# Ogeon/pyrite

Measured on AMD Instinct MI355X. Metric: Msamples/sec, higher is better.
Workload: dtype f32; 1 GPU; C3: c3_mesh_in_box, 1920x1080, 1024 spp; bounces=8, light_samples=4, spectrum_samples=10, spectrum_bins=64, tile_size=32, triangles=819212, spheres=0, parallelism=one launch on one GPU, film_weight_check=ok

## Files before the change

### pyrite_amd/build.py

```python
import os
import subprocess
import sys

CSRC = os.path.join(os.path.dirname(os.path.abspath(__file__)), "csrc")
OUT = os.path.join(CSRC, "libpyrite_gpu.so")
KERNELS = os.path.join(CSRC, "kernels")
KERNEL_UNITS = ["main.hip", "interp.hip", "product.hip", "wide.hip", "film.hip", "features.hip", "features_wide.hip", "tone.hip", "denoise.hip", "build.hip", "refit.hip"]
PROFILE_UNIT = "profile.hip"
PLAIN_UNITS = ["film.hip", "features.hip", "features_wide.hip", "tone.hip", "denoise.hip", "build.hip", "refit.hip"]
SOURCES = ["api.cpp", "multi.cpp", "bvh.cpp", "bvh_device.cpp", "program_regs.cpp"]
HEADERS = ["kernels.hip", "bvh.h", "bvh_level.h", "bvh_device.h", "device_scene.h", "api_internal.h", "exact_math.h", "program_regs.h", os.path.join("..", "..", "include", "pyrite_gpu.h")]
HIPCC = os.environ.get("HIPCC", "/opt/rocm/bin/hipcc")
FLAGS = [
    "-O3", "-std=c++17", "--offload-arch=gfx950", "-fPIC", "-shared",
    "-munsafe-fp-atomics",
    "-fno-fast-math",
    "-ffp-contract=off",
    "-Wall", "-Wno-unused-function",
    "-mllvm", "-disable-vector-combine",
    "-fno-slp-vectorize",
]


def stale():
    if not os.path.exists(OUT):
        return True
    t = os.path.getmtime(OUT)
    files = [os.path.join(CSRC, f) for f in SOURCES + HEADERS] + [os.path.join(KERNELS, f) for f in os.listdir(KERNELS)]
    return os.path.getmtime(os.path.abspath(__file__)) > t or any(os.path.getmtime(f) > t for f in files)


IMAGES_OUT = os.path.join(CSRC, "libpyrite_images.so")


def build_images(force=False, verbose=False):
    src = os.path.join(CSRC, "jpeg.c")
    if not force and os.path.exists(IMAGES_OUT) and os.path.getmtime(IMAGES_OUT) >= os.path.getmtime(src):
        return IMAGES_OUT
    cmd = [os.environ.get("CC", "gcc"), "-O2", "-fPIC", "-shared", "-Wall", "-o", IMAGES_OUT, src, "-lm"]
    if verbose:
        print(" ".join(cmd))
    subprocess.check_call(cmd, cwd=CSRC)
    return IMAGES_OUT

# ... 83 lines not shown
```

### pyrite_amd/csrc/device_scene.h

```cpp
#pragma once
#include <cstddef>
#include <cstdint>

#include "../../include/pyrite_gpu.h"

namespace pyr {

struct DevPrim {
    float a[4], b[4], c[4];
};

struct DevPrimPair {
    float q[5][4];
};

struct DevTriShade {
    float n1[4], n2[4], n3[4];
};

struct DevTriTex {
    float uv12[4], uv3[4], f1[4], f2[4], f3[4];
};

struct DevTexture {
// ... 88 lines not shown
constexpr uint32_t tape_rows_needed(uint32_t n_spectral, bool rgb) {
    return (rgb ? tape_rgb_row(n_spectral) + 3u : (n_spectral == 0u ? 0u : tape_row(n_spectral - 1u) + 1u)) > kTapeValueRows
               ? (rgb ? tape_rgb_row(n_spectral) + 3u : tape_row(n_spectral - 1u) + 1u)
               : kTapeValueRows;
}

constexpr uint32_t kMaxStackDepth = 64;

struct RenderLaunch {
    PyrCamera camera;
    PyrFilmDesc film;
    uint32_t bounces, light_samples, spectrum_samples, tile_size, pixel_samples;
    uint32_t tiles_x, tiles_y;
    uint32_t tile_begin, tile_stride, tile_count;
    uint32_t chunks_per_tile;
    uint32_t chunk_begin, chunk_end;
    uint32_t film_layout;
    uint32_t film_row_begin, film_row_count;
    uint64_t seed;
    float grains_per_wavelength;
    PyrGrain* film_out;
    unsigned long long* counters;
    uint32_t scheduler;
    uint32_t sm_phase_lanes, sm_trav_steps;
    uint32_t sm_expose_lanes;
    uint32_t stack_lds;
    unsigned long long* tape;
    uint32_t tape_lanes, tape_max_ops;
    uint32_t* tape_overflow;
    uint32_t tape_programs_lds;
    uint32_t sample_begin;
    uint32_t* start_queue;
    uint32_t start_queue_stride;
};

#ifndef PYR_SAMPLE_QUEUE
#define PYR_SAMPLE_QUEUE 1
#endif
constexpr uint32_t kStartQueueEntries = 128, kStartQueueFixedWords = 11;
constexpr uint32_t start_queue_words(uint32_t spectrum_samples) { return kStartQueueFixedWords + spectrum_samples; }

constexpr uint32_t kFeedSegments = 8, kFeedCursorStride = 64;
constexpr size_t kFeedBytes = (size_t)kFeedSegments * kFeedCursorStride * sizeof(uint32_t);

struct IntersectLaunch {
    const float* rays;
    PyrHit* hits;
    uint32_t n;
    unsigned long long* counters;
    uint32_t* next;
    uint32_t num_cus;
    uint32_t reserve;
    uint32_t stack_lds;
};

struct DevelopLaunch {
    PyrFilmDesc film;
    const PyrGrain* grains;
    float step_size, xyz_scale;
    uint32_t sample_count;
    const float* filter;
    const float* white_div;
    const float* white_mul;
    const float* xyz_table;
    uint32_t xyz_count;
    float xyz_min, xyz_max;
// ... 90 lines not shown
```

### pyrite_amd/csrc/kernels.hip

```cpp
#ifndef PYRITE_KERNELS_HIP
#define PYRITE_KERNELS_HIP
#include <hip/hip_runtime.h>

#include <algorithm>
#include <cstdint>
#include <cstdlib>
#include <string>
#include <type_traits>

#include "device_scene.h"
#include "exact_math.h"

#ifdef PYR_WIDE_VM
#define PYR_VM_NUMBERS PYR_WIDE_NUMBER_REGISTERS
#define PYR_VM_VECTORS PYR_WIDE_VECTOR_REGISTERS
#define PYR_VM_RGBS PYR_WIDE_RGB_REGISTERS
#else
#define PYR_VM_NUMBERS PYR_MAX_NUMBER_REGISTERS
#define PYR_VM_VECTORS PYR_MAX_VECTOR_REGISTERS
#define PYR_VM_RGBS PYR_MAX_RGB_REGISTERS
#endif
static_assert((PYR_VM_NUMBERS & (PYR_VM_NUMBERS - 1)) == 0 && (PYR_VM_VECTORS & (PYR_VM_VECTORS - 1)) == 0 && (PYR_VM_RGBS & (PYR_VM_RGBS - 1)) == 0,
              "the interpreter masks register indices: its files are powers of two");

namespace pyr {
#ifdef PYR_WIDE_VM
namespace wide {
#endif

#define DEV __device__ __forceinline__
DEV unsigned long long ballot64(bool p) { return __builtin_amdgcn_ballot_w64(p); }

constexpr int BLOCK = 256;
#ifndef PYR_SM_WAVES
#define PYR_SM_WAVES 4
#endif
constexpr float DIST_EPSILON = 0.0001f;
constexpr float PI_F = 3.14159265358979323846f;
#define PYR_INF __builtin_huge_valf()

struct f3 {
    float x, y, z;
};
DEV f3 mk(float x, float y, float z) { return f3{x, y, z}; }
// ... 1196 lines not shown
        spec.wl(hero) = spec.wl(SS - 1);
        if constexpr (COMPANION_STATE)
            for (uint32_t k = 0; k + 1 < SS; ++k) {
                spec.bright(k) = 0.0f;
                spec.refl(k) = 1.0f;
            }
    }
    p.bright = 0.0f;
    p.refl = 1.0f;
    p.use_additional = true;
    p.sample_light = true;
    p.events = 0;
    p.bounce = 0;
}

DEV bool locate_chunk(const RenderLaunch& L, uint32_t chunk, uint32_t lane, uint32_t& tile, uint64_t& iteration, TileArea& area) {
    const uint32_t k = chunk / L.chunks_per_tile, within = chunk - k * L.chunks_per_tile;
    tile = L.tile_begin + k * L.tile_stride;
    const uint32_t ty = tile / L.tiles_x, tx = tile - ty * L.tiles_x;
    const uint32_t sx = tx * L.tile_size, sy = ty * L.tile_size;
    const uint32_t w = min(L.film.width - sx, L.tile_size), h = min(L.film.height - sy, L.tile_size);
    const uint64_t area_px = (uint64_t)w * h, iterations = area_px * L.pixel_samples;
    iteration = (uint64_t)within * 64u + lane;
    if (iteration >= iterations) return false;
    iteration += area_px * L.sample_begin;
    area = to_view_area(sx, sy, w, h, L.film.width, L.film.height);
    return true;
}

struct SyncProf {
    unsigned long long section[8] = {0, 0, 0, 0, 0, 0, 0, 0}, last = 0;
};
#ifdef PYR_PHASE_PROFILE
__device__ unsigned long long g_phase_prof[16];
#define SLAP(sp, i)                                 \
    {                                               \
        const unsigned long long now_ = clock64();  \
        (sp).section[i] += now_ - (sp).last;        \
        (sp).last = now_;                           \
    }
#else
#define SLAP(sp, i)
#endif

constexpr int SYNC_PRIO_T = 3, SYNC_PRIO_N = 2, SYNC_PRIO_S = 1, SYNC_PRIO_E = 0;
#define SYNC_PRIO(x) __builtin_amdgcn_s_setprio(x)
template <bool COUNT>
DEV bool bounce_step(const DevScene& S, const RenderLaunch& L, const SceneView& view, Path& p, Spectral& spec, int* stack, Counters& cnt, SyncProf& sp) {
    const uint32_t n_add = L.spectrum_samples - 1;
    Hit hit;
    if (COUNT) cnt.extension_rays++;
    const f3 ray_o = p.o, ray_d = p.d;
    SYNC_PRIO(SYNC_PRIO_T);
    const bool found = traverse<COUNT, false>(S, view.nodes, view.prims, ray_o, ray_d, 0.0f, hit, stack, cnt);
    SYNC_PRIO(SYNC_PRIO_S);
    SLAP(sp, 1);
    if (!found) {
        uint32_t color = S.sky_program;
        if (p.sample_light) {
            for (uint32_t i = 0; i < S.num_lamps; ++i) {
                const DevLamp& l = S.lamps[i];
                if (l.kind == PYR_LAMP_DIRECTIONAL && dot(ld3(l.v), ray_d) >= l.width) {
                    color = l.color_program;
                    break;
                }
            }
        }
// ... 213 lines not shown
        uint32_t tile;
        uint64_t iteration;
        TileArea area;
        if (!locate_chunk(L, chunk, lane, tile, iteration, area)) continue;
        Path p{};
        start_sample(launch_from_kernarg(L), tile, iteration, area, p, spec);
        if (COUNT) cnt.samples++;
        SLAP(sp, 0);
        while (p.bounce < L.bounces) {
            const bool ended = bounce_step<COUNT>(S, launch_from_kernarg(L), view, p, spec, stack, cnt, sp);
            p.bounce++;
            if (ended) break;
        }
        SLAP(sp, 6);
        SYNC_PRIO(SYNC_PRIO_E);
        finish_path<COUNT>(launch_from_kernarg(L), p, spec, cnt);
        SLAP(sp, 7);
    }
#ifdef PYR_PHASE_PROFILE
    if (lane == 0)
        for (int i = 0; i < 8; ++i) atomicAdd(&g_phase_prof[i], sp.section[i]);
#endif
    flush_counters<COUNT>(cnt, L.counters);
}

#ifdef PYR_PHASE_PROFILE
#define PROF_DECL unsigned long long prof_c[4] = {0, 0, 0, 0}, prof_l[4] = {0, 0, 0, 0}, prof_n[4] = {0, 0, 0, 0}
#define PROF_BEGIN(ph, cond) const unsigned long long prof_t0_##ph = clock64(); prof_l[ph] += __popcll(ballot64(cond)); prof_n[ph]++
#define PROF_END(ph) prof_c[ph] += clock64() - prof_t0_##ph
#define PROF_LANES(ph, cond) prof_l[ph] += __popcll(ballot64(cond)); prof_n[ph]++
#define PROF_NOW() clock64()
#define PROF_EXTRA(idx, cycles) if ((threadIdx.x & 63u) == 0) atomicAdd(&g_phase_prof[idx], (unsigned long long)(cycles))
#define PROF_ADD(acc, v) (acc) += (v)
#define PROF_FLUSH()                                                                                  \
    if ((threadIdx.x & 63u) == 0)                                                                     \
        for (int i = 0; i < 4; ++i) {                                                                 \
            atomicAdd(&g_phase_prof[i], prof_c[i]);                                                   \
            atomicAdd(&g_phase_prof[4 + i], prof_l[i]);                                               \
            atomicAdd(&g_phase_prof[8 + i], prof_n[i]);                                               \
        }
#else
#define PROF_DECL
#define PROF_BEGIN(ph, cond)
#define PROF_END(ph)
#define PROF_LANES(ph, cond)
#define PROF_NOW() 0ull
#define PROF_EXTRA(idx, cycles)
#define PROF_ADD(acc, v)
#define PROF_FLUSH()
#endif

enum Stage : uint32_t { ST_NEW = 0, ST_TRAV = 1, ST_SHADE = 2, ST_NEE = 3, ST_EXPOSE = 4, ST_DONE = 5 };

struct Trav {
    f3 o, d, inv;
    uint32_t nx = 0, ny = 0, nz = 0;
    float limit, closest;
    int node, sp;
    uint32_t shape;
    float u, v;
    bool shadow, blocked;
};

DEV void trav_ray_signs(Trav& t) {
    t.nx = (__float_as_uint(t.d.x) >> 31) * 48u;
    t.ny = (__float_as_uint(t.d.y) >> 31) * 48u;
    t.nz = (__float_as_uint(t.d.z) >> 31) * 48u;
}
DEV float shadow_cutoff(float limit, float margin) { return __builtin_amdgcn_sqrtf(limit * margin + 1.0e-3f); }
DEV void trav_restart(Trav& t, float shadow_margin) {
    if (t.shadow) t.closest = shadow_cutoff(t.limit, shadow_margin);
    t.blocked = false;
    t.node = 0;
    t.sp = 0;
}

template <bool COUNT>
DEV bool trav_begin(const DevScene& S, Trav& t, f3 o, f3 d, bool shadow, float limit, Counters& cnt) {
    t.o = o;
    t.d = d;
    t.shadow = shadow;
// ... 339 lines not shown
    const uint32_t* tape_prepared = nullptr;
    DEV void tape_push(const RenderLaunch& L, uint32_t kind, uint32_t program, float s, bool hero_only = false) {
        if (n_ops < L.tape_max_ops) {
            uint32_t word = (kind << 30) | (hero_only ? TAPE_HERO_ONLY : 0u) | (program & TAPE_PROGRAM_MASK);
            if (tape_prepared != nullptr) {
                uint32_t slot = kTapeOneSlot;
                if (kind != TAPE_SCALE) {
                    const uint32_t* e = tape_prepared + 8 * program;
                    if (e[0] == 0u)
                        s = __uint_as_float(e[1]) * s;
                    else
                        slot = e[7];
                }
                word = (kind == TAPE_ADD ? TAPE_EAGER_ADD : 0u) | (hero_only ? TAPE_HERO_ONLY : 0u) | (slot << TAPE_EAGER_SLOT_SHIFT);
            }
            L.tape[tape_index(n_ops, L.tape_lanes, tape_column)] = (unsigned long long)word | ((unsigned long long)__float_as_uint(s) << 32);
        } else {
            *L.tape_overflow = 1u;
        }
        n_ops++;
    }
    DEV void tape_push_raw(const RenderLaunch& L, uint32_t word, float s) {
        if (n_ops < L.tape_max_ops)
            L.tape[tape_index(n_ops, L.tape_lanes, tape_column)] = (unsigned long long)word | ((unsigned long long)__float_as_uint(s) << 32);
        else
            *L.tape_overflow = 1u;
        n_ops++;
    }
    uint32_t rgb_slot = 0;
    static constexpr bool QUEUE = PYR_SAMPLE_QUEUE != 0 && TAPE && !INTERP;
    uint32_t chunk = 0;
    uint32_t q_state = 0;
#ifdef PYR_PHASE_PROFILE
    unsigned long long prof_start[4] = {0, 0, 0, 0};
#endif
    Path p{};
    Trav t{};
    f3 b_position = mk(0, 0, 0), b_normal = mk(0, 0, 0), b_out = mk(0, 0, 0);
    bool b_flip = false;
    DEV f3 b_nff() const { return b_flip ? -b_normal : b_normal; }
    bool b_has_brdf = false;
    uint32_t nee_lamp = 0, nee_i = 0;
    DEV static float nee_probability(const DevScene& S, const RenderLaunch& L) {
        const float lamp_probability = 1.0f / (float)S.num_lamps;
        return 1.0f / ((float)L.light_samples * 2.0f * PI_F * lamp_probability);
    }
    bool ls_pending = false, ls_physical = false;
    uint32_t ls_material = 0, ls_color = 0;
    f3 ls_normal = mk(0, 0, 0);
    float ls_scale = 0.0f;
    float ls_tx = 0.0f, ls_ty = 0.0f;

    enum : uint32_t { CONTRIB_NONE = 0, CONTRIB_MUL = 1, CONTRIB_ADD = 2 };
    uint32_t c_kind = CONTRIB_NONE, c_color = 0;
    int c_probability = -1;
    float c_cp = 1.0f, c_outer = 1.0f, c_scale = 1.0f;
    bool c_use_outer = false, c_companions = false, c_has_scale = false;
    f3 c_normal = mk(0, 0, 0), c_incident = mk(0, 0, 0);
    float c_tx = 0.0f, c_ty = 0.0f;
    DEV void contribution(uint32_t kind, uint32_t color, int probability, float cp, bool use_outer, float outer, bool companions, f3 normal, f3 incident, float tx,
                          float ty) {
        c_kind = kind, c_color = color, c_probability = probability, c_cp = cp, c_use_outer = use_outer, c_outer = outer, c_companions = companions;
        c_normal = normal, c_incident = incident, c_tx = tx, c_ty = ty;
    }
    DEV void contribution_clear() {
        c_kind = CONTRIB_NONE, c_color = 0u, c_probability = -1;
// ... 460 lines not shown
    for (uint32_t k = 0; k < p.num_instrs; ++k) {
        const PyrInstr& ins = S.instrs[p.first_instr + k];
        float r = 0.0f;
        switch (ins.op) {
        case PYR_OP_NUMBER: r = __uint_as_float(ins.x.bits); break;
        case PYR_OP_SPECTRUM: r = spectrum_get(S, ins.a, value(ins.x)); break;
        case PYR_OP_BLACKBODY: {
            const float wl = value(ins.x), temp = value(ins.y);
            r = blackbody(wl, temp);
            break;
        }
        case PYR_OP_MIX: {
            const float amount = fmaxf(fminf(value(ins.x), 1.0f), 0.0f);
            const float l = num[ins.a & (PYR_MAX_NUMBER_REGISTERS - 1)], rr = num[ins.b & (PYR_MAX_NUMBER_REGISTERS - 1)];
            r = l * (1.0f - amount) + rr * amount;
            break;
        }
        case PYR_OP_BINARY: {
            const float l = num[ins.a & (PYR_MAX_NUMBER_REGISTERS - 1)], rr = num[ins.b & (PYR_MAX_NUMBER_REGISTERS - 1)];
            r = ins.operator_ == PYR_BIN_ADD ? l + rr : (ins.operator_ == PYR_BIN_SUB ? l - rr : (ins.operator_ == PYR_BIN_MUL ? l * rr : l / rr));
            break;
        }
        default: {
            const float v = value(ins.x), mn = value(ins.y), mx = value(ins.z);
            r = fmaxf(fminf(v, mx), mn);
            break;
        }
        }
        num[ins.output & (PYR_MAX_NUMBER_REGISTERS - 1)] = r;
    }
    return num[p.output_reg & (PYR_MAX_NUMBER_REGISTERS - 1)];
}

template <bool COUNT, bool RGB = false, bool TIMES = false>
DEV void replay_tapes(const DevScene& S, const RenderLaunch& L, bool exposing, uint32_t n_ops, uint32_t tape_column, const Path& p, const float* wl_rows,
                      uint32_t wl_column, uint32_t* wave_list, const uint32_t* prepared_lds, float* spectral_values, uint32_t n_spectral, bool eager, Counters& cnt) {
    const uint32_t lane = threadIdx.x & 63u;
    const unsigned long long mask = ballot64(exposing);
    const uint32_t n = (uint32_t)__popcll(mask);
    if (n == 0) return;
    uint32_t max_ops = exposing ? (n_ops < L.tape_max_ops ? n_ops : L.tape_max_ops) : 0u;
    const uint32_t my_ops = max_ops;
    for (int off = 32; off > 0; off >>= 1) max_ops = max(max_ops, (uint32_t)__shfl_xor((int)max_ops, off));
    const bool keeps = exposing && p.use_additional, lost = exposing && !p.use_additional;
    const bool longest = 3u * my_ops > 2u * max_ops, shortest = 3u * my_ops <= max_ops;
    const unsigned long long below = (1ull << lane) - 1ull;
    const unsigned long long k0 = ballot64(keeps && longest), k1 = ballot64(keeps && !longest && !shortest), k2 = ballot64(keeps && shortest);
    const unsigned long long l0 = ballot64(lost && longest), l1 = ballot64(lost && !longest && !shortest), l2 = ballot64(lost && shortest);
    const uint32_t n_full = (uint32_t)__builtin_popcountll(k0 | k1 | k2);
    if (exposing) {
        const unsigned long long mine = keeps ? (longest ? k0 : (shortest ? k2 : k1)) : (longest ? l0 : (shortest ? l2 : l1));
        uint32_t before = keeps ? 0u : n_full;
        before += (uint32_t)__builtin_popcountll(keeps ? ((longest ? 0ull : k0) | (shortest ? k1 : 0ull)) : ((longest ? 0ull : l0) | (shortest ? l1 : 0ull)));
        wave_list[before + (uint32_t)__builtin_popcountll(mine & below)] = lane;
    }
    __builtin_amdgcn_wave_barrier();
    const uint32_t SS = L.spectrum_samples, full_items = n_full * SS, items = full_items + (n - n_full);
    const unsigned long long past_the_end =
        eager ? ((unsigned long long)(kTapeOneSlot << TAPE_EAGER_SLOT_SHIFT) | ((unsigned long long)__float_as_uint(1.0f) << 32)) : 0ull;
#ifndef PYR_REPLAY_ROWS
#define PYR_REPLAY_ROWS 8
#endif
    constexpr uint32_t ROWS = PYR_REPLAY_ROWS;
    for (uint32_t base = 0; base < items; base += 64) {
        const uint32_t i = base + lane;
        const bool active = i < items;
        const bool full = i < full_items;
        const uint32_t rank = !active ? 0u : (full ? i / SS : n_full + (i - full_items)), k = !active ? 0u : (full ? i - rank * SS : SS - 1u);
        const uint32_t src = wave_list[rank];
        const uint32_t ops = (uint32_t)__shfl((int)n_ops, (int)src);
        uint32_t pass_ops = active ? (ops < L.tape_max_ops ? ops : L.tape_max_ops) : 0u;
        for (int off = 32; off > 0; off >>= 1) pass_ops = max(pass_ops, (uint32_t)__shfl_xor((int)pass_ops, off));
        const uint32_t pixel = (uint32_t)__shfl((int)p.pixel, (int)src);
        const float hero_wl = __shfl(p.wl, (int)src);
        const bool hero = k == SS - 1;
        const bool run = active;
        const uint32_t src_column = (uint32_t)__shfl((int)wl_column, (int)src);
        const float wl = hero ? hero_wl : wl_rows[k * BLOCK + src_column];
        float refl = 1.0f, bright = 0.0f, value = 0.0f;
        uint32_t value_of = 0xFFFFFFFFu;
        [[maybe_unused]] float rgb_sum = 0.0f;
        if (eager) {
            const uint32_t* slot_program = prepared_lds + 8 * L.tape_programs_lds;
            uint32_t grid_min = 0, grid_max = 0, grid_count = 0;
            uint32_t i0 = 0, i1 = 0;
            float mix = 0.0f;
            bool below = false, above = false;
            for (uint32_t slot = 0; slot < n_spectral; ++slot) {
                const uint32_t* e = prepared_lds + 8 * slot_program[slot];
                const uint32_t mode = e[0], format = e[2], count = e[6];
                const float c = __uint_as_float(e[1]);
                const float* data = S.spectrum_data + e[5];
                float v;
                if (RGB && mode == 0xFFu) {
                    v = lambda_eval(S, S.programs[slot_program[slot]], wl);
                } else if (format == PYR_SPECTRUM_ARRAY && count != 0u) {
                    if (e[3] != grid_min || e[4] != grid_max || count != grid_count) {
                        grid_min = e[3], grid_max = e[4], grid_count = count;
                        const float lo = __uint_as_float(grid_min), hi = __uint_as_float(grid_max);
                        below = wl <= lo, above = wl >= hi;
                        const float normalized = (wl - lo) / (hi - lo);
                        const float float_index = normalized * ((float)count - 1.0f);
                        const float min_float_index = truncf(float_index);
                        i0 = (below | above) ? 0u : (uint32_t)min_float_index;
                        i1 = (below | above) ? 0u : i0 + 1u;
                        mix = float_index - min_float_index;
                    }
                    const float inside = data[i0] * (1.0f - mix) + data[i1] * mix;
                    v = below ? data[0] : (above ? data[count - 1] : inside);
                } else {
                    PyrSpectrum sp;
                    sp.format = format, sp.min = __uint_as_float(e[3]), sp.max = __uint_as_float(e[4]), sp.offset = e[5], sp.count = count;
                    v = spectrum_eval(sp, data, wl);
                }
                spectral_values[tape_row(slot) * BLOCK] = (mode == FAST_SPECTRUM || mode == 0xFFu) ? v : v * c;
            }
            if (RGB && S.rgb_records != 0) {
                float resp[3] = {0.0f, 0.0f, 0.0f};
                const uint32_t count = S.rgb_count;
                if (count > 0) {
                    const float* d = S.rgb_basis;
                    if (wl <= S.rgb_min) {
                        for (int j = 0; j < 3; ++j) resp[j] = d[j];
                    } else if (wl >= S.rgb_max) {
                        for (int j = 0; j < 3; ++j) resp[j] = d[3 * (count - 1) + j];
                    } else {
                        const float normalized = (wl - S.rgb_min) / (S.rgb_max - S.rgb_min);
                        const float fi = normalized * ((float)count - 1.0f);
                        const float fmin_ = truncf(fi);
                        const uint32_t b0 = (uint32_t)fmin_;
                        const float bmix = fi - fmin_;
                        for (int j = 0; j < 3; ++j) resp[j] = d[3 * b0 + j] * (1.0f - bmix) + d[3 * (b0 + 1) + j] * bmix;
                    }
                }
                for (uint32_t j = 0; j < 3; ++j) spectral_values[(tape_rgb_row(n_spectral) + j) * BLOCK] = resp[j];
            }
        }
        for (uint32_t r0 = 0; r0 < pass_ops; r0 += ROWS) {
            unsigned long long rows[ROWS];
#pragma unroll
            for (uint32_t j = 0; j < ROWS; ++j) rows[j] = r0 + j < my_ops ? L.tape[tape_index(r0 + j, L.tape_lanes, tape_column)] : past_the_end;
            uint32_t words[ROWS];
            float factors[ROWS];
#pragma unroll
            for (uint32_t j = 0; j < ROWS; ++j) {
                words[j] = (uint32_t)__shfl((int)(uint32_t)rows[j], (int)src);
                factors[j] = __uint_as_float((uint32_t)__shfl((int)(uint32_t)(rows[j] >> 32), (int)src));
            }
            if (eager) {
                float values[ROWS];
#pragma unroll
                for (uint32_t j = 0; j < ROWS; ++j) values[j] = spectral_values[words[j] & TAPE_EAGER_SLOT_MASK];
                if (RGB && (TIMES ? S.micro_records : S.rgb_records) != 0) {
                    const uint32_t not_mine = hero ? 0u : TAPE_HERO_ONLY;
#pragma unroll
                    for (uint32_t j = 0; j < ROWS; ++j) {
                        const float m = values[j] * factors[j];
                        const uint32_t op = (words[j] >> TAPE_RGB_SHIFT) & (TIMES ? 7u : 3u);
                        if constexpr (TIMES)
                            rgb_sum = op == 1u ? m : (op == 2u ? rgb_sum + m : (op == 4u ? rgb_sum * m : rgb_sum));
                        else
                            rgb_sum = op == 1u ? m : (op == 2u ? rgb_sum + m : rgb_sum);
                        const float mm = op == 3u ? rgb_sum * factors[j] : m;
                        const bool apply = ((words[j] & not_mine) == 0u) & ((op == 0u) | (op == 3u));
                        const bool adds = (int)words[j] < 0;
                        const float multiplied = refl * mm, added = bright + multiplied;
                        bright = (apply & adds) ? added : bright;
                        refl = (apply & !adds) ? multiplied : refl;
                    }
                    continue;
                }
                if (S.hero_only_records == 0) {
#pragma unroll
                    for (uint32_t j = 0; j < ROWS; ++j) {
                        const float m = values[j] * factors[j];
                        const bool adds = (int)words[j] < 0;
                        const float multiplied = refl * m, added = bright + multiplied;
                        bright = adds ? added : bright;
                        refl = adds ? refl : multiplied;
                    }
                    continue;
                }
                const uint32_t not_for_me = hero ? 0u : TAPE_HERO_ONLY;
#pragma unroll
                for (uint32_t j = 0; j < ROWS; ++j) {
                    const float m = values[j] * factors[j];
                    const bool apply = (words[j] & not_for_me) == 0u;
                    const bool adds = (int)words[j] < 0;
                    const float multiplied = refl * m, added = bright + multiplied;
                    bright = (apply & adds) ? added : bright;
                    refl = (apply & !adds) ? multiplied : refl;
                }
                continue;
            }
#pragma unroll
            for (uint32_t j = 0; j < ROWS; ++j) {
                const uint32_t word = words[j];
                const float s = factors[j];
                if (!run || r0 + j >= ops) continue;
                const uint32_t kind = word >> 30;
                if (kind == TAPE_SCALE) {
                    refl *= s;
                    continue;
                }
                if ((word & TAPE_HERO_ONLY) && !hero) continue;
                const uint32_t program = word & TAPE_PROGRAM_MASK;
                if (program != value_of) {
                    Prepared q_prog;
                    if (program < L.tape_programs_lds) {
                        const uint32_t* e = prepared_lds + 8 * program;
                        q_prog.mode = e[0];
                        q_prog.c = __uint_as_float(e[1]);
                        q_prog.sp.format = e[2];
                        q_prog.sp.min = __uint_as_float(e[3]);
                        q_prog.sp.max = __uint_as_float(e[4]);
                        q_prog.sp.offset = e[5];
                        q_prog.sp.count = e[6];
                        q_prog.data = S.spectrum_data + e[5];
                        q_prog.id = program;
                    } else {
                        q_prog = prepare_program<false>(S, program);
                    }
                    VmInput in{wl, mk(0, 0, 0), mk(0, 0, 0)};
                    value = eval_prepared<false>(S, q_prog, in);
                    value_of = program;
                }
                if (kind == TAPE_MUL)
                    refl *= value * s;
                else
// ... 76 lines not shown
    uint32_t* prepared_lds = reinterpret_cast<uint32_t*>(lds + lds_base_floats + (LDS_SCENE ? (S0.num_nodes * 16 + S0.num_prims * 12) : 0) + (LDS_TABLES ? S0.lds_table_floats : 0));
    uint32_t n_spectral = 0;
    bool eager = false;
    float* spectral_values = lds + (SS + 1) * BLOCK + threadIdx.x;
    if constexpr (TAPE) {
        spectral_values[kTapeOneSlot * BLOCK] = 1.0f;
        n_spectral = prepare_tape_tables(S0, S, L, prepared_lds, eager);
        if (eager) w.tape_prepared = prepared_lds;
        w.rgb_slot = tape_rgb_row(n_spectral);
        w.tape_column = blockIdx.x * BLOCK + threadIdx.x;
        if (HIT_TAPE && !eager) *L.tape_overflow = 1u;
    }

    auto scene_view = [&](const RenderLaunch& Lp) {
        if (LDS_SCENE || INTERP) return S;
        const uint32_t rows = (TAPE ? Lp.spectrum_samples + 1 + S0.tape_value_rows : 3 * Lp.spectrum_samples) + Lp.stack_lds;
        return stage_tables<LDS_TABLES ? 1 : 0, false>(scene_from_kernarg(S0), lds, rows * BLOCK);
    };
    PROF_DECL;
    for (;;) {
        int nT = __popcll(ballot64(w.stage == ST_TRAV));
        int nS = __popcll(ballot64(w.stage == ST_SHADE));
        int nN = __popcll(ballot64(w.stage == ST_NEE));
        int nE = __popcll(ballot64(w.stage == ST_EXPOSE || w.stage == ST_NEW));
        if (max(max(nT, nS), max(nN, nE)) == 0) break;

        if (nE >= expose_lanes || nE == max(max(nT, nS), max(nN, nE))) {
            PHASE_PRIO(PYR_PRIO_E);
            PROF_BEGIN(0, w.stage == ST_EXPOSE || w.stage == ST_NEW);
            const RenderLaunch& Lp = launch_from_kernarg(L);
            const DevScene Sp = scene_view(Lp);
            if constexpr (TAPE) {
                [[maybe_unused]] const unsigned long long t_r0 = PROF_NOW();
                replay_tapes<COUNT, HIT_TAPE, PRODUCT>(Sp, Lp, w.stage == ST_EXPOSE, w.n_ops, w.tape_column, w.p, lds, threadIdx.x, wave_list, prepared_lds, spectral_values, n_spectral,
                                              HIT_TAPE ? eager : n_spectral != 0, cnt);
                PROF_ADD(w.prof_start[3], PROF_NOW() - t_r0);
            }
            w.expose_and_restart(Sp, Lp, spec, cnt, lane, total_waves);
            PROF_END(0);
            nT = __popcll(ballot64(w.stage == ST_TRAV));
            nS = __popcll(ballot64(w.stage == ST_SHADE));
            nE = 0;
        }
        if (nS >= phase_lanes || nS == max(max(nT, nS), max(nN, nE))) {
            PHASE_PRIO(PYR_PRIO_S);
            PROF_BEGIN(1, w.stage == ST_SHADE);
            const RenderLaunch& Lp = launch_from_kernarg(L);
            w.shade(scene_view(Lp), Lp, spec, cnt);
            PROF_END(1);
            nT = __popcll(ballot64(w.stage == ST_TRAV));
            nN = __popcll(ballot64(w.stage == ST_NEE));
            nE = __popcll(ballot64(w.stage == ST_EXPOSE || w.stage == ST_NEW));
            nS = 0;
        }
        if (nN >= phase_lanes || nN == max(max(nT, nS), max(nN, nE))) {
            PHASE_PRIO(PYR_PRIO_N);
            PROF_BEGIN(2, w.stage == ST_NEE);
            const RenderLaunch& Lp = launch_from_kernarg(L);
            w.next_event(scene_view(Lp), Lp, spec, cnt);
            PROF_END(2);
            nT = __popcll(ballot64(w.stage == ST_TRAV));
            nN = __popcll(ballot64(w.stage == ST_NEE));
            nE = __popcll(ballot64(w.stage == ST_EXPOSE || w.stage == ST_NEW));
        }
        if constexpr (INTERP) {
            const unsigned long long pending = ballot64(w.c_kind != 0u || w.c_has_scale);
            if (pending != 0ull) {
                [[maybe_unused]] const unsigned long long t_c0 = PROF_NOW();
// ... 3 lines not shown
                if constexpr (HIT_TAPE)
                    w.tape_pending(scene_view(Lp), Lp);
                else
                    w.contribute_pending(scene_view(Lp), Lp, spec);
                PROF_EXTRA(12, PROF_NOW() - t_c0);
            }
            w.contribution_clear();
        }
        if (nT >= phase_lanes || nT == max(max(nT, nS), max(nN, nE))) {
#ifdef PYR_PHASE_PROFILE
            const unsigned long long prof_t0_3 = clock64();
#endif
            PHASE_PRIO(PYR_PRIO_T);
            w.t.inv = box_reciprocal(w.t.d);
            trav_ray_signs(w.t);
            if (!LDS_SCENE && view.wide && view.pairs != nullptr) {
                for (int step = 0; step < trav_steps; ++step) {
                    PROF_LANES(3, w.stage == ST_TRAV);
                    if (trav_step_lean<COUNT>(view, w.t, stack, cnt, w.stage == ST_TRAV)) w.stage = w.t.shadow ? ST_NEE : ST_SHADE;
                }
            } else {
                for (int step = 0; step < trav_steps; ++step) {
                    PROF_LANES(3, w.stage == ST_TRAV);
                    if (trav_step_voted<COUNT, !LDS_SCENE>(view, w.t, stack, cnt, w.stage == ST_TRAV)) w.stage = w.t.shadow ? ST_NEE : ST_SHADE;
                }
            }
            PROF_END(3);
        }
    }
    PROF_FLUSH();
#ifdef PYR_PHASE_PROFILE
    if constexpr (!INTERP)
        for (int i = 0; i < 4; ++i) PROF_EXTRA(12 + i, w.prof_start[i]);
#endif
    flush_counters<COUNT>(cnt, L.counters);
}


struct WorkFeed {
    uint32_t next = 0, end = 0;
    uint32_t segment = 0, visited = 0;
    bool drained = false;
};
DEV uint32_t feed_segment_begin(uint32_t n, uint32_t segment) { return (uint32_t)(((uint64_t)n * segment / kFeedSegments) & ~63ull); }
DEV uint32_t feed_segment_end(uint32_t n, uint32_t segment) { return segment + 1 == kFeedSegments ? n : feed_segment_begin(n, segment + 1); }
DEV void feed_reserve(WorkFeed& f, uint32_t* cursors, uint32_t n, uint32_t reserve, uint32_t lane) {
    while (f.next == f.end && !f.drained) {
        const uint32_t begin = feed_segment_begin(n, f.segment), end = feed_segment_end(n, f.segment);
        uint32_t base = 0;
        if (lane == 0) base = atomicAdd(&cursors[f.segment * kFeedCursorStride], reserve);
        base = __shfl(base, 0, 64);
        if (base < end - begin) {
            f.next = begin + base;
            f.end = begin + min(base + reserve, end - begin);
        } else if (++f.visited == kFeedSegments) {
            f.drained = true;
        } else {
            f.segment = (f.segment + 1) % kFeedSegments;
        }
    }
}

#ifndef PYR_INTERSECT_PAIRS
#define PYR_INTERSECT_PAIRS 1
#endif
#ifndef PYR_INTERSECT_WAVES
// ... 76 lines not shown
```

### pyrite_amd/csrc/kernels/main.hip

```cpp
#include "../kernels.hip"

namespace pyr {

namespace {
thread_local std::string g_kernel_error;
}
const char* kernels_last_error() { return g_kernel_error.c_str(); }

__global__ __launch_bounds__(BLOCK) void develop_kernel(DevelopLaunch D) {
    const size_t pixels = (size_t)D.film.width * D.film.height;
    const uint32_t bins = D.film.bins;
    const float min = D.film.wl_start, max = D.film.wl_start + D.film.wl_width;
    for (size_t px = (size_t)blockIdx.x * BLOCK + threadIdx.x; px < pixels; px += (size_t)gridDim.x * BLOCK) {
        uint8_t out[3] = {0, 0, 0};
        if ((px + 1) * bins < pixels * bins) {
            const PyrGrain* g = D.grains + px * bins;
            auto xyz_get = [&](int channel, float w) {
                const float* d = D.xyz_table;
                const uint32_t n = D.xyz_count;
                if (w <= D.xyz_min) return d[channel];
                if (w >= D.xyz_max) return d[3 * (n - 1) + channel];
                float normalized = (w - D.xyz_min) / (D.xyz_max - D.xyz_min);
                float fi = normalized * ((float)n - 1.0f);
                float fmin_ = truncf(fi);
// ... 162 lines not shown
    size_t bytes = (spectral_rows + launch.stack_lds) * BLOCK * sizeof(float);
    if (scene_fits_lds(scene)) bytes += (size_t)scene.num_nodes * 64 + (size_t)scene.num_prims * 48;
    bytes += (size_t)scene.lds_table_floats * sizeof(float);
    if (uses_tape(scene, launch)) bytes += ((size_t)tape_programs_in_lds(scene) * 8 + kTapeMaxValueRows) * sizeof(uint32_t);
    return bytes;
}


static RenderKernel pick_kernel(bool sm, bool with_counters, bool interp, bool lds_scene, bool lds_tables, bool hit_tape, bool product, bool wide_vm) {
    if (interp && wide_vm) return pick_wide_kernel(with_counters, lds_scene, lds_tables);
    if (interp) return pick_interp_kernel(with_counters, lds_scene, lds_tables, hit_tape, product);
    auto pick = [&](auto counters) -> RenderKernel {
        constexpr bool C = decltype(counters)::value;
        if (lds_scene) return sm ? render_kernel_sm<C, false, true, false> : render_kernel<C, true, false>;
        if (sm) return lds_tables ? render_kernel_sm<C, false, false, true> : render_kernel_sm<C, false, false, false>;
        return lds_tables ? render_kernel<C, false, true> : render_kernel<C, false, false>;
    };
    return with_counters ? pick(std::true_type{}) : pick(std::false_type{});
}

bool scene_is_lds_resident(const DevScene& scene) { return scene_fits_lds(scene); }

int launch_render(const DevScene& scene, const RenderLaunch& launch_in, bool with_counters, void* stream, int num_cus, bool wide_vm) {
    if (scene.stack_depth > kMaxStackDepth) {
        g_kernel_error = "BVH deeper than kMaxStackDepth";
        return PYR_ERR_UNSUPPORTED;
    }
    if (wide_vm && (launch_in.scheduler != 1 || scene.needs_interpreter == 0 || uses_tape(scene, launch_in))) {
        g_kernel_error = "the wide interpreter build runs the stage scheduler's online form only";
        return PYR_ERR_INVALID_ARGUMENT;
    }
    RenderLaunch launch = launch_in;
    launch.stack_lds = 0;
    launch.tape_programs_lds = uses_tape(scene, launch) ? tape_programs_in_lds(scene) : 0u;
    launch.stack_lds = launch.scheduler == 1 ? short_stack_levels(scene, render_lds_bytes(scene, launch), (uint32_t)sm_waves(scene.needs_interpreter != 0))
                                             : scene.stack_depth;
    if (scene_fits_lds(scene)) launch.stack_lds = std::max(launch.stack_lds, scene.stack_depth);
    const size_t lds = render_lds_bytes(scene, launch);
    if (lds > 160 * 1024) {
        g_kernel_error = "spectrum_samples + BVH depth need more than 160 KB of LDS per workgroup";
        return PYR_ERR_UNSUPPORTED;
    }
    const uint32_t chunks = launch.chunk_end - launch.chunk_begin;
    if (chunks == 0) return PYR_OK;
    RenderKernel kernel = pick_kernel(launch.scheduler == 1, with_counters, scene.needs_interpreter != 0, scene_fits_lds(scene), scene.lds_table_floats != 0,
                                      launch.scheduler == 1 && uses_hit_tape(scene, launch), scene.product_records != 0, wide_vm);
    if (kernel == nullptr) {
        g_kernel_error = "a program of this scene needs the wide interpreter build, which this one-unit build of the kernels does not hold";
        return PYR_ERR_UNSUPPORTED;
    }
    hipError_t err = hipFuncSetAttribute(reinterpret_cast<const void*>(kernel), hipFuncAttributeMaxDynamicSharedMemorySize, (int)lds);
    if (err != hipSuccess) {
        g_kernel_error = std::string("hipFuncSetAttribute: ") + hipGetErrorString(err);
        return PYR_ERR_DEVICE;
    }
    hipFuncAttributes attr{};
    int blocks_per_cu = 4;
    if (hipFuncGetAttributes(&attr, reinterpret_cast<const void*>(kernel)) == hipSuccess && attr.numRegs > 0) {
        int regs = ((attr.numRegs + 7) / 8) * 8;
        blocks_per_cu = std::min(8, 512 / regs);
    }
    blocks_per_cu = std::max(1, std::min<int>(blocks_per_cu, (int)((160 * 1024) / std::max<size_t>(lds, 1))));
    uint32_t grid = (uint32_t)num_cus * (uint32_t)blocks_per_cu;
    const uint32_t path_waves = BLOCK / 64;
    uint32_t blocks_needed = (chunks + path_waves - 1) / path_waves;
    if (grid > blocks_needed) grid = blocks_needed;
// ... 53 lines not shown
```

### pyrite_amd/csrc/kernels/profile.hip

```cpp
#include "main.hip"
#include "interp.hip"
#include "product.hip"

namespace pyr {
RenderKernel pick_wide_kernel(bool, bool, bool) { return nullptr; }
}

extern "C" int pyr_debug_phase_profile(unsigned long long* out16, int reset) {
    if (hipDeviceSynchronize() != hipSuccess) return -1;
    if (hipMemcpyFromSymbol(out16, HIP_SYMBOL(pyr::g_phase_prof), 16 * sizeof(unsigned long long)) != hipSuccess) return -1;
    if (reset) {
        unsigned long long zero[16] = {};
        if (hipMemcpyToSymbol(HIP_SYMBOL(pyr::g_phase_prof), zero, sizeof(zero)) != hipSuccess) return -1;
    }
    return 0;
}
```

Before: 650.4 Msamples/s.

## Sort replay lanes exactly by tape length and trim partial row blocks

Replaces the three-bucket long/medium/short ordering of finished lanes with an exact descending sort by tape length, built from per-bit ballots, and packs lane and length into each wave-list entry. Each 64-item pass now reads its row count from the first entry (plus the boundary entry) instead of a shuffle-max reduction. It also stops processing rows past the pass length inside the last 8-row block and swaps integer division for a magic multiply. The aim is to cut idle lanes and wasted rows during tape replay, at the cost of extra ballots per replay and more branching in the unrolled loops. It also adds replay profiling counters.

```diff
diff --git a/pyrite_amd/build.py b/pyrite_amd/build.py
--- a/pyrite_amd/build.py
+++ b/pyrite_amd/build.py
@@ -9,7 +9,7 @@
 PROFILE_UNIT = "profile.hip"
 PLAIN_UNITS = ["film.hip", "features.hip", "features_wide.hip", "tone.hip", "denoise.hip", "build.hip", "refit.hip"]
 SOURCES = ["api.cpp", "multi.cpp", "bvh.cpp", "bvh_device.cpp", "program_regs.cpp"]
-HEADERS = ["kernels.hip", "bvh.h", "bvh_level.h", "bvh_device.h", "device_scene.h", "api_internal.h", "exact_math.h", "program_regs.h", os.path.join("..", "..", "include", "pyrite_gpu.h")]
+HEADERS = ["kernels.hip", "bvh.h", "bvh_level.h", "bvh_device.h", "device_scene.h", "api_internal.h", "exact_math.h", "replay_plan.h", "program_regs.h", os.path.join("..", "..", "include", "pyrite_gpu.h")]
 HIPCC = os.environ.get("HIPCC", "/opt/rocm/bin/hipcc")
 FLAGS = [
     "-O3", "-std=c++17", "--offload-arch=gfx950", "-fPIC", "-shared",
diff --git a/pyrite_amd/csrc/device_scene.h b/pyrite_amd/csrc/device_scene.h
--- a/pyrite_amd/csrc/device_scene.h
+++ b/pyrite_amd/csrc/device_scene.h
@@ -144,6 +144,7 @@
     uint32_t sample_begin;
     uint32_t* start_queue;
     uint32_t start_queue_stride;
+    uint32_t replay_div;
 };
 
 #ifndef PYR_SAMPLE_QUEUE
diff --git a/pyrite_amd/csrc/kernels.hip b/pyrite_amd/csrc/kernels.hip
--- a/pyrite_amd/csrc/kernels.hip
+++ b/pyrite_amd/csrc/kernels.hip
@@ -10,6 +10,7 @@
 
 #include "device_scene.h"
 #include "exact_math.h"
+#include "replay_plan.h"
 
 #ifdef PYR_WIDE_VM
 #define PYR_VM_NUMBERS PYR_WIDE_NUMBER_REGISTERS
@@ -1272,7 +1273,7 @@
     unsigned long long section[8] = {0, 0, 0, 0, 0, 0, 0, 0}, last = 0;
 };
 #ifdef PYR_PHASE_PROFILE
-__device__ unsigned long long g_phase_prof[16];
+__device__ unsigned long long g_phase_prof[24];
 #define SLAP(sp, i)                                 \
     {                                               \
         const unsigned long long now_ = clock64();  \
@@ -1552,6 +1553,7 @@
 #define PROF_NOW() clock64()
 #define PROF_EXTRA(idx, cycles) if ((threadIdx.x & 63u) == 0) atomicAdd(&g_phase_prof[idx], (unsigned long long)(cycles))
 #define PROF_ADD(acc, v) (acc) += (v)
+#define PROF_PTR(x) (x)
 #define PROF_FLUSH()                                                                                  \
     if ((threadIdx.x & 63u) == 0)                                                                     \
         for (int i = 0; i < 4; ++i) {                                                                 \
@@ -1567,6 +1569,7 @@
 #define PROF_NOW() 0ull
 #define PROF_EXTRA(idx, cycles)
 #define PROF_ADD(acc, v)
+#define PROF_PTR(x) nullptr
 #define PROF_FLUSH()
 #endif
 
@@ -1972,6 +1975,7 @@
     uint32_t chunk = 0;
     uint32_t q_state = 0;
 #ifdef PYR_PHASE_PROFILE
+    unsigned long long prof_replay[8] = {0, 0, 0, 0, 0, 0, 0, 0};
     unsigned long long prof_start[4] = {0, 0, 0, 0};
 #endif
     Path p{};
@@ -2498,27 +2502,43 @@
     return num[p.output_reg & (PYR_MAX_NUMBER_REGISTERS - 1)];
 }
 
-template <bool COUNT, bool RGB = false, bool TIMES = false>
+#ifndef PYR_REPLAY_EXACT
+#define PYR_REPLAY_EXACT 1
+#endif
+template <bool COUNT, bool RGB = false, bool TIMES = false, bool EXACT = false>
 DEV void replay_tapes(const DevScene& S, const RenderLaunch& L, bool exposing, uint32_t n_ops, uint32_t tape_column, const Path& p, const float* wl_rows,
-                      uint32_t wl_column, uint32_t* wave_list, const uint32_t* prepared_lds, float* spectral_values, uint32_t n_spectral, bool eager, Counters& cnt) {
+                      uint32_t wl_column, uint32_t* wave_list, const uint32_t* prepared_lds, float* spectral_values, uint32_t n_spectral, bool eager, Counters& cnt,
+                      [[maybe_unused]] unsigned long long* prof) {
     const uint32_t lane = threadIdx.x & 63u;
     const unsigned long long mask = ballot64(exposing);
     const uint32_t n = (uint32_t)__popcll(mask);
     if (n == 0) return;
-    uint32_t max_ops = exposing ? (n_ops < L.tape_max_ops ? n_ops : L.tape_max_ops) : 0u;
-    const uint32_t my_ops = max_ops;
-    for (int off = 32; off > 0; off >>= 1) max_ops = max(max_ops, (uint32_t)__shfl_xor((int)max_ops, off));
-    const bool keeps = exposing && p.use_additional, lost = exposing && !p.use_additional;
-    const bool longest = 3u * my_ops > 2u * max_ops, shortest = 3u * my_ops <= max_ops;
-    const unsigned long long below = (1ull << lane) - 1ull;
-    const unsigned long long k0 = ballot64(keeps && longest), k1 = ballot64(keeps && !longest && !shortest), k2 = ballot64(keeps && shortest);
-    const unsigned long long l0 = ballot64(lost && longest), l1 = ballot64(lost && !longest && !shortest), l2 = ballot64(lost && shortest);
-    const uint32_t n_full = (uint32_t)__builtin_popcountll(k0 | k1 | k2);
-    if (exposing) {
-        const unsigned long long mine = keeps ? (longest ? k0 : (shortest ? k2 : k1)) : (longest ? l0 : (shortest ? l2 : l1));
-        uint32_t before = keeps ? 0u : n_full;
-        before += (uint32_t)__builtin_popcountll(keeps ? ((longest ? 0ull : k0) | (shortest ? k1 : 0ull)) : ((longest ? 0ull : l0) | (shortest ? l1 : 0ull)));
-        wave_list[before + (uint32_t)__builtin_popcountll(mine & below)] = lane;
+    PROF_ADD(prof[0], 1);
+    PROF_ADD(prof[1], n);
+    const uint32_t my_ops = exposing ? replay_plan::tape_length(n_ops, L.tape_max_ops) : 0u;
+    const bool keeps = exposing && p.use_additional;
+    uint32_t n_full;
+    if constexpr (EXACT) {
+        const unsigned long long keepers = ballot64(keeps);
+        n_full = (uint32_t)__builtin_popcountll(keepers);
+        const uint32_t position =
+            replay_plan::list_position(lane, my_ops, keeps, mask, keepers, replay_plan::length_bits(L.tape_max_ops), [&](uint32_t b) { return ballot64(((my_ops >> b) & 1u) != 0u); });
+        if (exposing) wave_list[position] = replay_plan::list_entry(lane, my_ops);
+    } else {
+        uint32_t max_ops = my_ops;
+        for (int off = 32; off > 0; off >>= 1) max_ops = max(max_ops, (uint32_t)__shfl_xor((int)max_ops, off));
+        const bool lost = exposing && !p.use_additional;
+        const bool longest = 3u * my_ops > 2u * max_ops, shortest = 3u * my_ops <= max_ops;
+        const unsigned long long below = (1ull << lane) - 1ull;
+        const unsigned long long k0 = ballot64(keeps && longest), k1 = ballot64(keeps && !longest && !shortest), k2 = ballot64(keeps && shortest);
+        const unsigned long long l0 = ballot64(lost && longest), l1 = ballot64(lost && !longest && !shortest), l2 = ballot64(lost && shortest);
+        n_full = (uint32_t)__builtin_popcountll(k0 | k1 | k2);
+        if (exposing) {
+            const unsigned long long mine = keeps ? (longest ? k0 : (shortest ? k2 : k1)) : (longest ? l0 : (shortest ? l2 : l1));
+            uint32_t before = keeps ? 0u : n_full;
+            before += (uint32_t)__builtin_popcountll(keeps ? ((longest ? 0ull : k0) | (shortest ? k1 : 0ull)) : ((longest ? 0ull : l0) | (shortest ? l1 : 0ull)));
+            wave_list[before + (uint32_t)__builtin_popcountll(mine & below)] = lane;
+        }
     }
     __builtin_amdgcn_wave_barrier();
     const uint32_t SS = L.spectrum_samples, full_items = n_full * SS, items = full_items + (n - n_full);
@@ -2528,15 +2548,32 @@
 #define PYR_REPLAY_ROWS 8
 #endif
     constexpr uint32_t ROWS = PYR_REPLAY_ROWS;
+    static_assert(!EXACT || ROWS == replay_plan::kBlockRows, "replay_plan.h plans blocks of kBlockRows rows");
     for (uint32_t base = 0; base < items; base += 64) {
         const uint32_t i = base + lane;
         const bool active = i < items;
         const bool full = i < full_items;
-        const uint32_t rank = !active ? 0u : (full ? i / SS : n_full + (i - full_items)), k = !active ? 0u : (full ? i - rank * SS : SS - 1u);
-        const uint32_t src = wave_list[rank];
-        const uint32_t ops = (uint32_t)__shfl((int)n_ops, (int)src);
-        uint32_t pass_ops = active ? (ops < L.tape_max_ops ? ops : L.tape_max_ops) : 0u;
-        for (int off = 32; off > 0; off >>= 1) pass_ops = max(pass_ops, (uint32_t)__shfl_xor((int)pass_ops, off));
+        uint32_t rank, k, src, ops, pass_ops;
+        if constexpr (EXACT) {
+            const replay_plan::Item item = replay_plan::item_of(active ? i : 0u, n_full, SS, L.replay_div);
+            rank = item.rank, k = active ? item.k : 0u;
+            const uint32_t entry = wave_list[rank];
+            src = replay_plan::entry_lane(entry), ops = replay_plan::entry_length(entry);
+            pass_ops = (uint32_t)__builtin_amdgcn_readfirstlane(
+                (int)replay_plan::pass_rows(base, n, n_full, SS, L.replay_div, [&](uint32_t at) { return replay_plan::entry_length(wave_list[at]); }));
+        } else {
+            rank = !active ? 0u : (full ? i / SS : n_full + (i - full_items)), k = !active ? 0u : (full ? i - rank * SS : SS - 1u);
+            src = wave_list[rank];
+            ops = (uint32_t)__shfl((int)n_ops, (int)src);
+            pass_ops = active ? (ops < L.tape_max_ops ? ops : L.tape_max_ops) : 0u;
+            for (int off = 32; off > 0; off >>= 1) pass_ops = max(pass_ops, (uint32_t)__shfl_xor((int)pass_ops, off));
+        }
+        PROF_ADD(prof[2], 1);
+        PROF_ADD(prof[3], (items - base < 64u ? items - base : 64u));
+        PROF_ADD(prof[4], (EXACT ? pass_ops : (pass_ops + ROWS - 1u) / ROWS * ROWS));
+        PROF_ADD(prof[5], (active ? (ops < L.tape_max_ops ? ops : L.tape_max_ops) : 0u));
+        PROF_ADD(prof[6], (eager ? n_spectral : 0u));
+        PROF_ADD(prof[7], (pass_ops + ROWS - 1u) / ROWS);
         const uint32_t pixel = (uint32_t)__shfl((int)p.pixel, (int)src);
         const float hero_wl = __shfl(p.wl, (int)src);
         const bool hero = k == SS - 1;
@@ -2603,6 +2640,7 @@
             }
         }
         for (uint32_t r0 = 0; r0 < pass_ops; r0 += ROWS) {
+            const uint32_t here = EXACT ? replay_plan::rows_in_block(pass_ops, r0) : ROWS;
             unsigned long long rows[ROWS];
 #pragma unroll
             for (uint32_t j = 0; j < ROWS; ++j) rows[j] = r0 + j < my_ops ? L.tape[tape_index(r0 + j, L.tape_lanes, tape_column)] : past_the_end;
@@ -2621,6 +2659,7 @@
                     const uint32_t not_mine = hero ? 0u : TAPE_HERO_ONLY;
 #pragma unroll
                     for (uint32_t j = 0; j < ROWS; ++j) {
+                        if (EXACT && j >= here) break;
                         const float m = values[j] * factors[j];
                         const uint32_t op = (words[j] >> TAPE_RGB_SHIFT) & (TIMES ? 7u : 3u);
                         if constexpr (TIMES)
@@ -2639,6 +2678,7 @@
                 if (S.hero_only_records == 0) {
 #pragma unroll
                     for (uint32_t j = 0; j < ROWS; ++j) {
+                        if (EXACT && j >= here) break;
                         const float m = values[j] * factors[j];
                         const bool adds = (int)words[j] < 0;
                         const float multiplied = refl * m, added = bright + multiplied;
@@ -2650,6 +2690,7 @@
                 const uint32_t not_for_me = hero ? 0u : TAPE_HERO_ONLY;
 #pragma unroll
                 for (uint32_t j = 0; j < ROWS; ++j) {
+                    if (EXACT && j >= here) break;
                     const float m = values[j] * factors[j];
                     const bool apply = (words[j] & not_for_me) == 0u;
                     const bool adds = (int)words[j] < 0;
@@ -2661,6 +2702,7 @@
             }
 #pragma unroll
             for (uint32_t j = 0; j < ROWS; ++j) {
+                if (EXACT && j >= here) break;
                 const uint32_t word = words[j];
                 const float s = factors[j];
                 if (!run || r0 + j >= ops) continue;
@@ -2803,8 +2845,8 @@
             const DevScene Sp = scene_view(Lp);
             if constexpr (TAPE) {
                 [[maybe_unused]] const unsigned long long t_r0 = PROF_NOW();
-                replay_tapes<COUNT, HIT_TAPE, PRODUCT>(Sp, Lp, w.stage == ST_EXPOSE, w.n_ops, w.tape_column, w.p, lds, threadIdx.x, wave_list, prepared_lds, spectral_values, n_spectral,
-                                              HIT_TAPE ? eager : n_spectral != 0, cnt);
+                replay_tapes<COUNT, HIT_TAPE, PRODUCT, PYR_REPLAY_EXACT != 0 && !INTERP>(Sp, Lp, w.stage == ST_EXPOSE, w.n_ops, w.tape_column, w.p, lds, threadIdx.x, wave_list, prepared_lds, spectral_values, n_spectral,
+                                              HIT_TAPE ? eager : n_spectral != 0, cnt, PROF_PTR(w.prof_replay));
                 PROF_ADD(w.prof_start[3], PROF_NOW() - t_r0);
             }
             w.expose_and_restart(Sp, Lp, spec, cnt, lane, total_waves);
@@ -2874,6 +2916,13 @@
 #ifdef PYR_PHASE_PROFILE
     if constexpr (!INTERP)
         for (int i = 0; i < 4; ++i) PROF_EXTRA(12 + i, w.prof_start[i]);
+    if constexpr (TAPE)
+        for (int i = 0; i < 8; ++i) {
+            if (i == 5)
+                atomicAdd(&g_phase_prof[16 + i], w.prof_replay[i]);
+            else
+                PROF_EXTRA(16 + i, w.prof_replay[i]);
+        }
 #endif
     flush_counters<COUNT>(cnt, L.counters);
 }
diff --git a/pyrite_amd/csrc/kernels/main.hip b/pyrite_amd/csrc/kernels/main.hip
--- a/pyrite_amd/csrc/kernels/main.hip
+++ b/pyrite_amd/csrc/kernels/main.hip
@@ -218,6 +218,7 @@
     }
     RenderLaunch launch = launch_in;
     launch.stack_lds = 0;
+    launch.replay_div = replay_plan::div_magic(launch.spectrum_samples);
     launch.tape_programs_lds = uses_tape(scene, launch) ? tape_programs_in_lds(scene) : 0u;
     launch.stack_lds = launch.scheduler == 1 ? short_stack_levels(scene, render_lds_bytes(scene, launch), (uint32_t)sm_waves(scene.needs_interpreter != 0))
                                              : scene.stack_depth;
diff --git a/pyrite_amd/csrc/kernels/profile.hip b/pyrite_amd/csrc/kernels/profile.hip
--- a/pyrite_amd/csrc/kernels/profile.hip
+++ b/pyrite_amd/csrc/kernels/profile.hip
@@ -15,3 +15,13 @@
     }
     return 0;
 }
+
+extern "C" int pyr_debug_replay_profile(unsigned long long* out8, int reset) {
+    if (hipDeviceSynchronize() != hipSuccess) return -1;
+    if (hipMemcpyFromSymbol(out8, HIP_SYMBOL(pyr::g_phase_prof), 8 * sizeof(unsigned long long), 16 * sizeof(unsigned long long)) != hipSuccess) return -1;
+    if (reset) {
+        unsigned long long zero[8] = {};
+        if (hipMemcpyToSymbol(HIP_SYMBOL(pyr::g_phase_prof), zero, sizeof(zero), 16 * sizeof(unsigned long long)) != hipSuccess) return -1;
+    }
+    return 0;
+}
diff --git a/pyrite_amd/csrc/replay_plan.h b/pyrite_amd/csrc/replay_plan.h
--- /dev/null
+++ b/pyrite_amd/csrc/replay_plan.h
@@ -0,0 +1,84 @@
+#pragma once
+#include <cstdint>
+
+#if defined(__HIPCC__)
+#include <hip/hip_runtime.h>
+#define PYR_RP __host__ __device__ __forceinline__
+#else
+#define PYR_RP inline
+#endif
+
+namespace pyr {
+namespace replay_plan {
+
+constexpr uint32_t kLanes = 64;
+constexpr uint32_t kBlockRows = 8;
+
+PYR_RP uint32_t popcount64(unsigned long long m) { return (uint32_t)__builtin_popcountll(m); }
+
+PYR_RP uint32_t tape_length(uint32_t n_ops, uint32_t tape_max_ops) { return n_ops < tape_max_ops ? n_ops : tape_max_ops; }
+
+PYR_RP uint32_t length_bits(uint32_t tape_max_ops) { return tape_max_ops == 0u ? 0u : 32u - (uint32_t)__builtin_clz(tape_max_ops); }
+
+template <class BitVote>
+PYR_RP uint32_t list_position(uint32_t lane, uint32_t length, bool keeps, unsigned long long finished, unsigned long long keepers, uint32_t bits, BitVote bit_vote) {
+    unsigned long long level = keeps ? keepers : finished & ~keepers, ahead = 0ull;
+    for (uint32_t b = bits; b-- > 0u;) {
+        const unsigned long long set = bit_vote(b);
+        const bool mine = ((length >> b) & 1u) != 0u;
+        ahead |= mine ? 0ull : level & set;
+        level &= mine ? set : ~set;
+    }
+    const unsigned long long below = (1ull << lane) - 1ull;
+    return (keeps ? 0u : popcount64(keepers)) + popcount64(ahead) + popcount64(level & below);
+}
+
+constexpr uint32_t kEntryLengthShift = 8;
+PYR_RP uint32_t list_entry(uint32_t lane, uint32_t length) { return lane | (length << kEntryLengthShift); }
+PYR_RP uint32_t entry_lane(uint32_t entry) { return entry & (kLanes - 1u); }
+PYR_RP uint32_t entry_length(uint32_t entry) { return entry >> kEntryLengthShift; }
+
+PYR_RP uint32_t full_items(uint32_t n_full, uint32_t spectrum_samples) { return n_full * spectrum_samples; }
+PYR_RP uint32_t item_count(uint32_t n_finished, uint32_t n_full, uint32_t spectrum_samples) { return full_items(n_full, spectrum_samples) + (n_finished - n_full); }
+
+constexpr uint32_t kDivShift = 18, kDivMaxDivisor = 64, kDivMaxNumerator = kLanes * kDivMaxDivisor;
+PYR_RP uint32_t div_magic(uint32_t d) { return (1u << kDivShift) / d + 1u; }
+PYR_RP uint32_t div_by_magic(uint32_t i, uint32_t magic) {
+#if defined(__HIP_DEVICE_COMPILE__)
+    return __umul24(i, magic) >> kDivShift;
+#else
+    return (i * magic) >> kDivShift;
+#endif
+}
+struct Item {
+    uint32_t rank;
+    uint32_t k;
+};
+PYR_RP Item item_of(uint32_t i, uint32_t n_full, uint32_t spectrum_samples, uint32_t magic) {
+    const uint32_t full = full_items(n_full, spectrum_samples);
+    Item it;
+    if (i < full) {
+        it.rank = div_by_magic(i, magic);
+        it.k = i - it.rank * spectrum_samples;
+    } else {
+        it.rank = n_full + (i - full);
+        it.k = spectrum_samples - 1u;
+    }
+    return it;
+}
+
+template <class LengthAt>
+PYR_RP uint32_t pass_rows(uint32_t base, uint32_t n_finished, uint32_t n_full, uint32_t spectrum_samples, uint32_t magic, LengthAt length_at) {
+    const uint32_t full = full_items(n_full, spectrum_samples);
+    uint32_t rows = length_at(item_of(base, n_full, spectrum_samples, magic).rank);
+    if (base < full && base + kLanes > full && n_finished > n_full) {
+        const uint32_t behind = length_at(n_full);
+        rows = behind > rows ? behind : rows;
+    }
+    return rows;
+}
+PYR_RP uint32_t pass_blocks(uint32_t rows) { return (rows + kBlockRows - 1u) / kBlockRows; }
+PYR_RP uint32_t rows_in_block(uint32_t rows, uint32_t r0) { return rows - r0 < kBlockRows ? rows - r0 : kBlockRows; }
+
+}
+}
```

Result: no change. 656.6 Msamples/s, median of 6 (+1.0%).
